# reglab/aquaculture

Hardware: AMD Instinct MI355X
Metric: 640px tiles/sec (whole node) YOLOv5m bf16 (higher is better)
Workload: dtype bf16

## Files before the change

aquaculture_amd/csrc/conv1x1_direct.hip:

```cpp
#include "conv_device.h"

using namespace aqdev;

namespace {

struct C1Params {
    const char* in;
    char* out;
    const char* w;
    const float* bias;
    const char* zero;
    int in_ld_b, out_ld_b;
    int npix, n_tiles, act;
    float out_inv_scale;
};

constexpr int kNW = 12;

template <int KS, int MBT, int MBW, int NBW> struct C1Geom {
    static constexpr int CIN = 32 * KS, COUT = 16 * MBT, CB = CIN / 8;
    static constexpr int MG = MBT / MBW;
    static constexpr int PG = kNW / MG;
    static constexpr int TP = PG * NBW * 16;
    static constexpr int SPP = CB + 2;
    static constexpr int PXB = SPP * 16;
    static constexpr int NQ = (TP * SPP + 63) / 64;
    static constexpr int XPB = NQ * 1024;
    static constexpr int LDS = 2 * XPB + COUT * 4;
    static constexpr int NST = NBW;
    static_assert(MBT % MBW == 0 && kNW % MG == 0 && LDS <= 160 * 1024, "shape");
};

__device__ __forceinline__ f32x4 c1_silu4(f32x4 v) {
    const f32x4 t = v * -1.44269504f;
    f32x4 d = {__builtin_amdgcn_exp2f(t[0]), __builtin_amdgcn_exp2f(t[1]), __builtin_amdgcn_exp2f(t[2]), __builtin_amdgcn_exp2f(t[3])};
    d = d + 1.0f;
    const f32x4 r = {__builtin_amdgcn_rcpf(d[0]), __builtin_amdgcn_rcpf(d[1]), __builtin_amdgcn_rcpf(d[2]), __builtin_amdgcn_rcpf(d[3])};
    return v * r;
}

template <int KS, int MBT, int MBW, int NBW, bool F8OUT = false>
__global__ __launch_bounds__(kNW * 64) void conv1x1_direct_kernel(const C1Params p) {
    using G = C1Geom<KS, MBT, MBW, NBW>;
    extern __shared__ __attribute__((aligned(16))) char smem[];
    float* s_b = (float*)(smem + 2 * G::XPB);

    const int tid = threadIdx.x, lane = tid & 63;
    const int wave = __builtin_amdgcn_readfirstlane(tid >> 6);
    static_assert(MBW == 2, "the paired-row layout below is written for two M blocks per wave");
    const int mb0 = (wave % G::MG) * MBW, pg = wave / G::MG;
    const int g = lane >> 4, l15 = lane & 15;
    const int cbase = mb0 * 16 + g * 8;

    bf16x8 wv[KS][MBW];
#pragma unroll
    for (int s = 0; s < KS; ++s)
#pragma unroll
        for (int m = 0; m < MBW; ++m) wv[s][m] = ((const bf16x8*)p.w)[((size_t)(mb0 + m) * KS + s) * 64 + lane];
    for (int i = tid; i < G::COUT; i += kNW * 64) s_b[i] = p.bias[i];

    auto issue_dma = [&](int tile, char* xb) {
        const long long n0 = (long long)tile * G::TP;
#pragma unroll 1
        for (int q = wave; q < G::NQ; q += kNW) {
            const int slot = q * 64 + lane;
            const int px = slot / G::SPP, part = slot - px * G::SPP;
            const bool valid = px < G::TP && part < G::CB && n0 + px < p.npix;
            const char* src = p.in + (n0 + px) * p.in_ld_b + part * 16;
            glds16(valid ? src : p.zero, xb + q * 1024);
        }
    };

    int tile = first_tile(gridDim.x, blockIdx.x);
    if (tile < p.n_tiles) issue_dma(tile, smem);
    int cur = 0;
    bool prev_full = false;
    for (; tile < p.n_tiles; tile += gridDim.x, cur ^= 1) {
        const long long n0 = (long long)tile * G::TP;
        const char* s_x = smem + cur * G::XPB;
        if (prev_full) wait_vmcnt<G::NST>(); else wait_vmcnt<0>();
        asm volatile("s_waitcnt lgkmcnt(0)" ::: "memory");
        __builtin_amdgcn_s_barrier();
        asm volatile("" ::: "memory");
        prev_full = n0 + G::TP <= p.npix;
        if (tile + (int)gridDim.x < p.n_tiles) issue_dma(tile + (int)gridDim.x, smem + (cur ^ 1) * G::XPB);

        f32x4 bv[MBW];
#pragma unroll
        for (int m = 0; m < MBW; ++m) bv[m] = *(const f32x4*)(s_b + cbase + m * 4);
        static_assert(G::NST == NBW * 1, "one 16-byte (8-byte with F8OUT) store per pixel block: the wait at the top of the tile loop counts these");
        AQ_STORE_LOOP_UNROLL
// ... 11 lines not shown
#pragma unroll
                for (int m = 0; m < MBW; ++m) acc[m] = __builtin_amdgcn_mfma_f32_16x16x32_bf16(wv[s][m], f[s], acc[m], 0, 0, 0);
            f32x4 v0 = acc[0] + bv[0], v1 = acc[1] + bv[1];
            if (p.act) { v0 = c1_silu4(v0); v1 = c1_silu4(v1); }
            if constexpr (F8OUT) {
                f32x4 q0 = v0 * p.out_inv_scale, q1 = v1 * p.out_inv_scale;
#pragma unroll
                for (int e = 0; e < 4; ++e) {
                    q0[e] = __builtin_amdgcn_fmed3f(q0[e], -448.0f, 448.0f);
                    q1[e] = __builtin_amdgcn_fmed3f(q1[e], -448.0f, 448.0f);
                }
                int w0 = __builtin_amdgcn_cvt_pk_fp8_f32(q0[0], q0[1], 0, false);
                w0 = __builtin_amdgcn_cvt_pk_fp8_f32(q0[2], q0[3], w0, true);
                int w1 = __builtin_amdgcn_cvt_pk_fp8_f32(q1[0], q1[1], 0, false);
                w1 = __builtin_amdgcn_cvt_pk_fp8_f32(q1[2], q1[3], w1, true);
                if (n0 + px < p.npix) *(uint2*)(p.out + (n0 + px) * p.out_ld_b + cbase) = make_uint2((unsigned)w0, (unsigned)w1);
            } else if (n0 + px < p.npix)
                *(uint4*)(p.out + (n0 + px) * p.out_ld_b + cbase * 2) =
                    make_uint4(pack_bf16x2(v0[0], v0[1]), pack_bf16x2(v0[2], v0[3]), pack_bf16x2(v1[0], v1[1]), pack_bf16x2(v1[2], v1[3]));
        }
    }
}

template <int KS, int MBT, int MBW, int NBW, bool F8OUT = false>
int launch_c1(C1Params p, hipStream_t stream) {
    using G = C1Geom<KS, MBT, MBW, NBW>;
    auto fn = conv1x1_direct_kernel<KS, MBT, MBW, NBW, F8OUT>;
    int cus = 0;
    AQ_CHECK_HIP(aq_kernel_lds((const void*)fn, G::LDS));
    AQ_CHECK_HIP(aq_cus(&cus));
    p.n_tiles = (p.npix + G::TP - 1) / G::TP;
    long long grid = cus;
    if (grid > p.n_tiles) grid = p.n_tiles;
    hipLaunchKernelGGL(fn, dim3((unsigned)grid), dim3(kNW * 64), G::LDS, stream, p);
    AQ_CHECK_HIP(hipGetLastError());
    return AQ_OK;
}

}

extern "C" int aq_conv1x1_direct_supported(int cin, int cout) {
    return (cin == 96 && cout == 96) || (cin == 192 && cout == 192) || (cin == 384 && (cout == 192 || cout == 384));
}

extern "C" int aq_pack_conv1x1_direct(const float* w_host, int cin, int cout, void* packed_dev, size_t* bytes, void* stream) {
    AQ_REQUIRE(w_host && bytes && aq_conv1x1_direct_supported(cin, cout), "pack_conv1x1_direct: unsupported %d -> %d", cin, cout);
    const int ks = cin / 32, mbt = cout / 16;
    *bytes = (size_t)mbt * ks * 64 * 16;
    if (!packed_dev) return AQ_OK;
    bf16_t* host = (bf16_t*)calloc(1, *bytes);
    AQ_REQUIRE(host, "pack_conv1x1_direct: out of host memory");
    for (int mb = 0; mb < mbt; ++mb)
        for (int s = 0; s < ks; ++s)
            for (int lane = 0; lane < 64; ++lane) {
                const int r = lane & 15, g = lane >> 4;
                const int co = (mb >> 1) * 32 + 8 * (r >> 2) + 4 * (mb & 1) + (r & 3);
                bf16_t* dst = host + (((size_t)mb * ks + s) * 64 + lane) * 8;
                for (int e = 0; e < 8; ++e) dst[e] = aq_f2bf(w_host[(size_t)co * cin + 32 * s + 8 * g + e]);
            }
// ... 5 lines not shown
}

extern "C" int aq_conv1x1_direct(const void* in_dev, int in_ld, int in_choff, void* out_dev, int out_ld, int out_choff, int cin, int cout,
                                 const void* packed_w_dev, const float* bias_dev, long long npix, int act, void* stream) {
    AQ_REQUIRE(in_dev && out_dev && packed_w_dev && bias_dev, "conv1x1_direct: null pointer");
    AQ_REQUIRE(aq_conv1x1_direct_supported(cin, cout), "conv1x1_direct: unsupported %d -> %d", cin, cout);
    AQ_REQUIRE(npix > 0 && npix < (1LL << 31), "conv1x1_direct: bad pixel count");
    AQ_REQUIRE(in_ld % 8 == 0 && out_ld % 8 == 0 && in_choff % 8 == 0 && out_choff % 8 == 0 && in_choff + cin <= in_ld && out_choff + cout <= out_ld,
               "conv1x1_direct: channel slices must be 8-aligned and inside their rows");
    C1Params p{};
    p.in = (const char*)in_dev + (size_t)in_choff * 2; p.in_ld_b = in_ld * 2;
    p.out = (char*)out_dev + (size_t)out_choff * 2; p.out_ld_b = out_ld * 2;
    p.w = (const char*)packed_w_dev; p.bias = bias_dev;
    p.npix = (int)npix; p.act = act;
    p.zero = aq_zero_page();
    AQ_REQUIRE(p.zero, "conv1x1_direct: zero page allocation failed");
    const hipStream_t st = (hipStream_t)stream;
    if (cin == 96) return launch_c1<3, 6, 2, 4>(p, st);
    if (cin == 192) return launch_c1<6, 12, 2, 4>(p, st);
    if (cout == 192) return launch_c1<12, 12, 2, 2>(p, st);
    return launch_c1<12, 24, 2, 4>(p, st);
}


extern "C" int aq_conv1x1_direct_f8out(const void* in_dev, int in_ld, int in_choff, void* out_dev, int out_pitch_bytes, int out_byte_off, int cin,
                                       int cout, const void* packed_w_dev, const float* bias_dev, long long npix, int act, float out_scale,
                                       void* stream) {
    AQ_REQUIRE(in_dev && out_dev && packed_w_dev && bias_dev, "conv1x1_direct_f8out: null pointer");
    AQ_REQUIRE((cin == 192 && cout == 192) || (cin == 384 && cout == 384), "conv1x1_direct_f8out: unsupported %d -> %d", cin, cout);
    AQ_REQUIRE(npix > 0 && npix < (1LL << 31) && out_scale > 0.0f, "conv1x1_direct_f8out: bad pixel count or scale");
    AQ_REQUIRE(in_ld % 8 == 0 && in_choff % 8 == 0 && in_choff + cin <= in_ld && out_pitch_bytes % 8 == 0 && out_byte_off % 8 == 0 &&
                   out_byte_off + cout <= out_pitch_bytes, "conv1x1_direct_f8out: slices must be 8-byte aligned and inside their rows");
    C1Params p{};
    p.in = (const char*)in_dev + (size_t)in_choff * 2; p.in_ld_b = in_ld * 2;
    p.out = (char*)out_dev + out_byte_off; p.out_ld_b = out_pitch_bytes;
    p.w = (const char*)packed_w_dev; p.bias = bias_dev;
    p.npix = (int)npix; p.act = act; p.out_inv_scale = 1.0f / out_scale;
    p.zero = aq_zero_page();
    AQ_REQUIRE(p.zero, "conv1x1_direct_f8out: zero page allocation failed");
    const hipStream_t st = (hipStream_t)stream;
    if (cin == 192) return launch_c1<6, 12, 2, 4, true>(p, st);
    return launch_c1<12, 24, 2, 4, true>(p, st);
}
```

aquaculture_amd/csrc/engine.cpp:

```cpp
#include "aq_common.h"
#include <unistd.h>
#include <string>

#include <cstdarg>
#include <cstdio>
#include <cstdlib>
#include <cstring>
#include <string>
#include <atomic>
#include <dlfcn.h>
#include <vector>

namespace {
thread_local char g_err[512] = "";
}

void aq_set_error(const char* fmt, ...) {
    va_list ap;
    va_start(ap, fmt);
    vsnprintf(g_err, sizeof(g_err), fmt, ap);
    va_end(ap);
}

extern "C" const char* aq_last_error(void) { return g_err; }
// ... 25 lines not shown
        return push && pop;
    }
} g_roctx;

constexpr int kCountStride = 1024;

struct PackedW {
    void* w = nullptr;
    float* bias = nullptr;
    int kgroups = 0, kgroups_pad = 0, G = 0, cout_rows = 0;
    bool x3 = false;
    void* w_direct = nullptr;
    int direct_cfg = -1;
    void* w_head = nullptr;
    void* w_pl8 = nullptr;
    float* sb_pl8 = nullptr;
    void* w_f8 = nullptr;
    float* sb_f8 = nullptr;
    float act_scale = 0.0f;
    int f8_consumer = -1;
    std::vector<float> w_host, b_host;
    void* w_tail = nullptr;
    float* b_tail = nullptr;
};

void pack_host(const float* w, int cout, int k, int cin, int precision, std::vector<unsigned char>& out,
               int* kgroups, int* kgroups_pad, int* G, int* cout_rows) {
    const int eb = aq_elem_bytes(precision);
    const int g = cin * eb / 16;
    const int kg = k * k * g;
    const int kgp = (kg + 7) / 8 * 8;
    const int rows = (cout + kCoutSlack + 31) / 32 * 32;
    out.assign((size_t)rows * kgp * 16, 0);
    const int kelems = k * k * cin;
    for (int co = 0; co < cout; ++co) {
        unsigned char* dst = out.data() + (size_t)co * kgp * 16;
        const float* src = w + (size_t)co * kelems;
        if (precision == AQ_FP32) {
            memcpy(dst, src, (size_t)kelems * 4);
        } else {
            bf16_t* d = (bf16_t*)dst;
            for (int e = 0; e < kelems; ++e) d[e] = aq_f2bf(src[e]);
        }
    }
    *kgroups = kg; *kgroups_pad = kgp; *G = g; *cout_rows = rows;
}
// ... 376 lines not shown
        }
        default:
            break;
        }
    }
    return -1;
}

bool c3tail_active(aq_engine* e, int oi, int last, int B) {
    if (!e->packed[oi].w_tail || oi + 1 >= last || e->calib_amax || e->tuning) return false;
    const int ci = oi + 1;
    const PackedW& pc = e->packed[ci];
    if (pc.direct_cfg != AQ_CONV_CFG_DIRECT1X1 || (pc.f8_consumer >= 0 && f8_pair_active(e, pc.f8_consumer, B))) return false;
    const aq_engine::Tuned* tt = tuned_for(e);
    const int cfg = e->conv_cfg[ci] >= 0 ? e->conv_cfg[ci] : tt ? tt->cfg[ci] : -1;
    if (cfg != AQ_CONV_CFG_DIRECT1X1) return false;
    const aq_op_desc& b = e->ops[oi];
    const aq_op_desc& c = e->ops[ci];
    const TensorPlace& pl = e->place[b.src.tensor];
    return aq_bottleneck_c3tail_supported(B, pl.h, pl.w, e->tensors[b.src.tensor].channels, e->tensors[c.src.tensor].channels,
                                          e->tensors[c.dst.tensor].channels) != 0;
}

struct AugRun {
    int pass;
    const aq_augment_pass* ps;
    int H0, W0;
    const aq_tap* ytab;
    const aq_tap* xtab;
};

int run_plan(aq_engine* e, const uint8_t* tiles, int B, int H, int W, void* ws, size_t ws_bytes,
             float* pred_out, aq_det* dets, int32_t* counts, float conf, float iou, int max_det, hipStream_t stream,
             int first = 0, int last = -1, const AugRun* ar = nullptr) {
    AQ_REQUIRE(e && tiles && ws, "infer: null pointer");
    const int n_ops = (int)e->ops.size();
    if (last < 0) last = n_ops;
    AQ_REQUIRE(0 <= first && first <= last && last <= n_ops, "run_ops: range [%d, %d) is not inside the plan's %d ops", first, last, n_ops);
    int rc = AQ_OK;
    if (!ar) {
        rc = layout(e, B, H, W);
        if (rc) return rc;
        if (ws_bytes < e->total_bytes) {
            aq_set_error("workspace too small: need %zu bytes, got %zu", e->total_bytes, ws_bytes);
            return AQ_ERR_WORKSPACE;
        }
// ... 3 lines not shown
    const float aug_scale = ar ? ar->ps->scale : 1.0f, aug_flip_w = ar && ar->ps->flip ? (float)ar->W0 : 0.0f;
    e->last_ws = ws; e->last_tiles = tiles;
    const int prec = e->desc.precision;
    const bool whole = first == 0 && last == n_ops;
    hipEvent_t* ev = nullptr;
    if (whole && !ar && e->prof && e->ring > 0) ev = e->ev.data() + (size_t)(e->prof_calls % e->ring) * (n_ops + 1);
    float* pred = pred_out ? pred_out : (float*)((char*)ws + e->off_pred);
    int32_t* cand = (int32_t*)((char*)ws + e->off_cand);
    int32_t* cand_count = (int32_t*)((char*)ws + e->off_cand_count);
    float* cand_rows = (float*)((char*)ws + e->off_cand_rows);
    const char* use_sd = getenv("AQ_STEMDOWN");
    const bool stemdown = use_sd && *use_sd == '1' && prec == AQ_BF16 && n_ops > 2 && e->ops[0].kind == AQ_OP_STEM && e->ops[1].kind == AQ_OP_DOWNBLOCK &&
                          e->ops[0].dst.channels == 48 && e->ops[1].src.tensor == e->ops[0].dst.tensor && e->ops[1].src.ch_off == e->ops[0].dst.ch_off &&
                          aq_stemdown_supported(H, W) && ((uintptr_t)tiles & 3) == 0 && !scaled;
    const bool fuse_heads = dets != nullptr && heads_fused(e);
    bool heads_started = ar != nullptr;
    int heads_done = 0;
    for (int oi = 0; oi < first; ++oi)
        if (fuse_heads && e->ops[oi].kind == AQ_OP_CONV && e->ops[oi].level >= 0) {
            heads_started = true;
            ++heads_done;
        }
    int tail_conv = -1;
    for (int oi = first; oi < last; ++oi) {
        const aq_op_desc& op = e->ops[oi];
        if (ev) AQ_CHECK_HIP(hipEventRecord(ev[oi], stream));
        const bool mark = g_roctx.on();
        if (mark) {
            char name[96];
            snprintf(name, sizeof name, "aq op %02d kind %d: %d -> %d ch, k%d s%d%s", oi, op.kind, op.src.channels, op.dst.channels, op.k, op.stride,
                     op.level >= 0 ? " (detect head)" : "");
            g_roctx.push(name);
        }
        switch (op.kind) {
        case AQ_OP_PREPROCESS:
            if (scaled)
                rc = aq_preprocess_s2d_scaled(tiles, ar->H0, ar->W0, ar->ytab, ar->xtab, ar->ps->h, ar->ps->w, tptr(e, ws, tiles, op.dst.tensor), B, H, W,
                                              prec, stream);
            else
                rc = aq_preprocess_s2d(tiles, tptr(e, ws, tiles, op.dst.tensor), B, H, W, prec, stream);
            break;
        case AQ_OP_CONV:
            if (oi == tail_conv) {
                note_launch(e, oi, AQ_FAM_DIRECT1X1, AQ_CONV_CFG_DIRECT1X1);
                break;
            }
            if (ar && op.level >= 0 && !((ar->ps->level_mask >> op.level) & 1)) {
                note_launch(e, oi, AQ_FAM_NONE);
                break;
            }
            if (fuse_heads && op.level >= 0) {
                int32_t* wide = (int32_t*)((char*)ws + e->off_cand_wide);
                if (!heads_started) {
                    AQ_CHECK_HIP(hipMemsetAsync(wide, 0, sizeof(int32_t) * B * kCountStride, stream));
                    heads_started = true;
                }
                const TensorPlace& pl = e->place[op.src.tensor];
                int off = 0;
                for (int l = 0; l < op.level; ++l) off += e->desc.na * (H / (int)e->desc.stride[l]) * (W / (int)e->desc.stride[l]);
                float anchors[8 * 2];
                for (int a = 0; a < e->desc.na; ++a) {
                    anchors[2 * a] = e->desc.anchors_px[op.level][a][0];
                    anchors[2 * a + 1] = e->desc.anchors_px[op.level][a][1];
                }
                note_launch(e, oi, AQ_FAM_HEAD_DECODE);
                if (ar) {
                    rc = aq_head_decode_aug(tptr(e, ws, tiles, op.src.tensor), e->tensors[op.src.tensor].channels, op.src.ch_off, op.src.channels,
// ... 45 lines not shown
                               op.src.channels, e->packed[oi].w, e->packed[oi].bias, B, pl.h, pl.w, op.res.tensor >= 0, stream);
            break;
        }
        case AQ_OP_DOWNBLOCK: {
            note_launch(e, oi, AQ_FAM_DOWNBLOCK);
            const TensorPlace& pl = e->place[op.src.tensor];
            if (stemdown && oi == 1) {
                rc = aq_stemdown(tiles, tptr(e, ws, tiles, op.dst.tensor), e->tensors[op.dst.tensor].channels, op.dst.ch_off,
                                 e->packed[0].w, e->packed[0].bias, e->packed[oi].w, e->packed[oi].bias, B, H, W, stream);
                break;
            }
            rc = aq_downblock(tptr(e, ws, tiles, op.src.tensor), e->tensors[op.src.tensor].channels, op.src.ch_off,
                              tptr(e, ws, tiles, op.dst.tensor), e->tensors[op.dst.tensor].channels, op.dst.ch_off,
                              e->packed[oi].w, e->packed[oi].bias, B, pl.h, pl.w, stream);
            break;
        }
        case AQ_OP_SPPF_POOL: {
            const TensorPlace& pl = e->place[op.src.tensor];
            rc = aq_sppf_pool(tptr(e, ws, tiles, op.src.tensor), e->tensors[op.src.tensor].channels, op.src.ch_off,
                              op.src.channels, B, pl.h, pl.w, prec, stream);
            break;
        }
        case AQ_OP_UPSAMPLE2X: {
            const TensorPlace& pl = e->place[op.src.tensor];
            rc = aq_upsample2x(tptr(e, ws, tiles, op.src.tensor), e->tensors[op.src.tensor].channels, op.src.ch_off,
                               tptr(e, ws, tiles, op.dst.tensor), e->tensors[op.dst.tensor].channels, op.dst.ch_off,
                               op.src.channels, B, pl.h, pl.w, prec, stream);
            break;
        }
        case AQ_OP_DECODE: {
            if (fuse_heads) break;
            const float* heads[3];
            for (int l = 0; l < 3; ++l) heads[l] = (const float*)tptr(e, ws, tiles, e->desc.head_tensor[l]);
            float anchors[3 * 8 * 2];
            for (int l = 0; l < 3; ++l)
                for (int a = 0; a < e->desc.na; ++a) {
                    anchors[(l * e->desc.na + a) * 2] = e->desc.anchors_px[l][a][0];
                    anchors[(l * e->desc.na + a) * 2 + 1] = e->desc.anchors_px[l][a][1];
                }
            const bool want_nms = dets != nullptr;
            if (ar) {
                rc = aq_detect_decode_aug(heads, e->tensors[e->desc.head_tensor[0]].channels, B, H, W, e->desc.nc, e->desc.na, anchors,
                                          e->desc.stride, ar->ps->level_mask, aug_base, e->N, aug_scale, aug_flip_w, want_nms ? nullptr : pred,
                                          conf, want_nms ? cand : nullptr, want_nms ? cand_rows : nullptr, want_nms ? cand_count : nullptr,
                                          e->N, stream);
                break;
// ... 370 lines not shown
                        (void)hipFree(pw.w_pl8); (void)hipFree(pw.sb_pl8);
                        pw.w_pl8 = nullptr; pw.sb_pl8 = nullptr;
                    }
                }
            }
        }
        const char* no_hf = getenv("AQ_DISABLE_HEAD_FUSION");
        if (d->precision == AQ_BF16 && op.level >= 0 && op.k == 1 && op.stride == 1 && !op.act && op.res.tensor < 0 &&
            op.dst.channels >= d->na * (d->nc + 5) && op.dst.channels <= 32 && aq_head_decode_supported(op.src.channels, d->na, d->nc) && !(no_hf && *no_hf == '1')) {
            size_t nb = 0;
            if (aq_pack_head_weights(op.weight, op.bias, op.src.channels, op.dst.channels, nullptr, &nb, nullptr) != AQ_OK ||
                hipMalloc(&pw.w_head, nb) != hipSuccess ||
                aq_pack_head_weights(op.weight, op.bias, op.src.channels, op.dst.channels, pw.w_head, &nb, nullptr) != AQ_OK) {
                aq_set_error("engine_create: fused head weight upload failed (op %zu)", oi);
                return fail(AQ_ERR_HIP);
            }
        }
        if (d->precision == AQ_BF16 && op.kind == AQ_OP_CONV && op.k == 3 && op.stride == 1 && op.pad == 1 && e->packed[oi].direct_cfg == AQ_CONV_CFG_PL3X3 &&
            aq_conv3x3_pl_f8_supported(op.src.channels, op.dst.channels, 1, 8, 8)) {
            e->packed[oi].w_host.assign(op.weight, op.weight + (size_t)op.dst.channels * 9 * op.src.channels);
            e->packed[oi].b_host.assign(op.bias, op.bias + op.dst.channels);
        }
        op.weight = nullptr; op.bias = nullptr;
    }
    *out = e;
    return AQ_OK;
}

extern "C" void aq_engine_destroy(aq_engine* e) {
    if (!e) return;
    for (PackedW& pw : e->packed) {
        if (pw.w) (void)hipFree(pw.w);
        if (pw.w_direct) (void)hipFree(pw.w_direct);
        if (pw.w_head) (void)hipFree(pw.w_head);
        if (pw.w_pl8) (void)hipFree(pw.w_pl8);
        if (pw.w_f8) (void)hipFree(pw.w_f8);
        if (pw.sb_f8) (void)hipFree(pw.sb_f8);
        if (pw.sb_pl8) (void)hipFree(pw.sb_pl8);
        if (pw.w_tail) (void)hipFree(pw.w_tail);
        if (pw.b_tail) (void)hipFree(pw.b_tail);
        if (pw.bias) (void)hipFree(pw.bias);
    }
    if (e->zero_page) (void)hipFree(e->zero_page);
    for (hipEvent_t ev : e->ev) (void)hipEventDestroy(ev);
    delete e;
}
// ... 328 lines not shown
```

aquaculture_amd/engine.py:

```python
from __future__ import annotations

import ctypes as C
import os
import re
from typing import Dict, List, Optional, Sequence, Tuple

import numpy as np
import torch

from . import spec as _spec
from .checkpoint import Checkpoint, pack_plan_weights

AQ_BF16, AQ_FP32, AQ_BF16_W8, AQ_F16X3 = 0, 1, 2, 3
PRECISIONS = {"bf16": AQ_BF16, "fp32": AQ_FP32, "fp8w": AQ_BF16, "f16x3": AQ_F16X3}
"""Compute precision of the single-op helpers.  fp8w = fp8 (OCP e4m3fn) weights with per-output-channel power-of-two scales, bf16
activations (quant.py): values bf16 holds exactly, so every bf16 kernel runs them as they are."""
ENGINE_PRECISIONS = {"bf16": AQ_BF16, "fp32": AQ_FP32, "fp8w": AQ_BF16_W8, "f16x3": AQ_F16X3, "fp8": AQ_BF16}
"""aq_model_desc.precision.  AQ_BF16_W8 computes as AQ_BF16; kernels with an fp8-weight stream (the planar 3x3) load the e4m3 codes."""
_DTYPE_CODE = {"act": 0, "f32": 1, "u8": 2}

LIB_PATH = os.path.join(os.path.dirname(os.path.abspath(__file__)), "csrc", "libaqengine.so")


class aq_tensor_desc(C.Structure):
# ... 9 lines not shown
                ("k", C.c_int32), ("stride", C.c_int32), ("pad", C.c_int32), ("act", C.c_int32),
                ("level", C.c_int32), ("weight", C.POINTER(C.c_float)), ("bias", C.POINTER(C.c_float)),
                ("flops_per_tile", C.c_double)]


class aq_model_desc(C.Structure):
    _fields_ = [("precision", C.c_int32), ("nc", C.c_int32), ("na", C.c_int32), ("nl", C.c_int32),
                ("anchors_px", C.c_float * 2 * 8 * 3), ("stride", C.c_float * 3),
                ("head_tensor", C.c_int32 * 3), ("input_tensor", C.c_int32),
                ("n_tensors", C.c_int32), ("n_ops", C.c_int32),
                ("tensors", C.POINTER(aq_tensor_desc)), ("ops", C.POINTER(aq_op_desc))]


class aq_det(C.Structure):
    _fields_ = [("x1", C.c_float), ("y1", C.c_float), ("x2", C.c_float), ("y2", C.c_float),
                ("conf", C.c_float), ("cls", C.c_float)]


EXPORTS = (
    "aq_last_error", "aq_version", "aq_engine_create", "aq_engine_destroy", "aq_engine_workspace_bytes",
    "aq_engine_infer", "aq_engine_run_ops", "aq_engine_candidates", "aq_engine_forward_raw", "aq_engine_tensor_ptr", "aq_engine_profile",
    "aq_engine_op_times", "aq_engine_num_ops", "aq_engine_set_conv_config", "aq_engine_autotune", "aq_engine_set_tuned_table",
    "aq_engine_get_conv_config", "aq_conv_num_configs", "aq_debug_conv_stamp", "aq_debug_mfma_peak",
    "aq_conv_config_tiles", "aq_pack_conv_weights", "aq_pack_conv_weights_x3", "aq_conv2d", "aq_pack_stem_weights", "aq_stem_conv", "aq_pack_bottleneck_weights", "aq_bottleneck", "aq_bottleneck_asm_form", "aq_bottleneck_c3tail_supported", "aq_pack_bottleneck_c3tail_weights", "aq_bottleneck_c3tail", "aq_pack_downblock_weights", "aq_downblock", "aq_stemdown_supported", "aq_stemdown", "aq_conv1x1_direct_supported", "aq_pack_conv1x1_direct", "aq_conv1x1_direct", "aq_conv1x1_asm_supported", "aq_pack_conv1x1_asm", "aq_conv1x1_asm", "aq_nms_opts", "aq_engine_set_nms_options",
    "aq_conv3x3s2_direct_supported", "aq_pack_conv3x3s2_direct", "aq_conv3x3s2_direct",
    "aq_conv3x3_pl_supported", "aq_conv3x3_pl_asm_family", "aq_pack_conv3x3_pl", "aq_conv3x3_pl", "aq_conv3x3_pl_s2_supported", "aq_pack_conv3x3_pl_s2", "aq_conv3x3_pl_s2", "aq_jpeg_scratch_bytes", "aq_jpeg_idct_rgb", "aq_f32_to_e4m3", "aq_conv1x1_direct_f8out", "aq_absmax_bf16", "aq_engine_calibrate_amax", "aq_engine_set_fp8_scales", "aq_engine_last_launch", "aq_conv3x3_pl_f8_supported", "aq_pack_conv3x3_pl_f8", "aq_conv3x3_pl_f8", "aq_conv3x3_pl_w8_supported", "aq_pack_conv3x3_pl_w8", "aq_conv3x3_pl_w8", "aq_head_decode_supported", "aq_pack_head_weights", "aq_head_decode", "aq_head_counts_gather", "aq_preprocess_s2d", "aq_sppf_pool",
    "aq_upsample2x", "aq_letterbox_u8", "aq_letterbox_tiles_u8", "aq_format_label_rows", "aq_detect_decode", "aq_nms_scratch_bytes", "aq_nms", "aq_jpeg_huffman_decode", "aq_write_label_files",
    "aq_crop_jpeg_coefs", "aq_crop_jpeg_bytes", "aq_write_crop_files",
    "aq_annotate_u8", "aq_image_jpeg_coefs", "aq_image_jpeg_bytes", "aq_write_image_files",
    "aq_blank_stats_scratch_bytes", "aq_blank_stats_u8",
    "aq_augment_geometry", "aq_augment_taps", "aq_stem_conv_scaled", "aq_preprocess_s2d_scaled", "aq_head_decode_aug", "aq_detect_decode_aug",
    "aq_engine_workspace_bytes_augment", "aq_engine_infer_augment", "aq_engine_forward_raw_augment", "aq_engine_last_launch_augment",
)

_lib = None


def load_library(path: str = LIB_PATH) -> C.CDLL:
    global _lib
    if _lib is not None:
        return _lib
    if path == LIB_PATH and os.environ.get("AQ_ENGINE_LIB"):
        path = os.environ["AQ_ENGINE_LIB"]
    if not os.path.exists(path):
        raise RuntimeError(f"{path} not found: build it with `python -m aquaculture_amd.build` "
                           "(there is no CPU/PyTorch fallback for the detect path)")
    lib = C.CDLL(path)
# ... 37 lines not shown
    lib.aq_engine_set_fp8_scales.argtypes = [vp, C.POINTER(f32), i32]
    lib.aq_conv1x1_direct_f8out.argtypes = [vp, i32, i32, vp, i32, i32, i32, i32, vp, vp, C.c_longlong, i32, f32, vp]
    lib.aq_absmax_bf16.argtypes = [vp, i32, i32, i32, C.c_longlong, vp, vp]
    lib.aq_debug_conv_stamp.argtypes = [vp, sz]
    lib.aq_debug_mfma_peak.argtypes = [i32, i32, vp, vp]
    lib.aq_conv_config_tiles.argtypes = [i32, C.POINTER(i32), C.POINTER(i32)]
    lib.aq_pack_conv_weights.argtypes = [C.POINTER(f32), i32, i32, i32, i32, vp, C.POINTER(sz), vp]
    lib.aq_pack_conv_weights_x3.argtypes = [C.POINTER(f32), C.POINTER(f32), i32, i32, i32, vp, C.POINTER(sz), vp, C.POINTER(sz), vp]
    lib.aq_conv2d.argtypes = [vp, i32, i32, i32, vp, i32, i32, i32, vp, i32, i32, vp, vp,
                              i32, i32, i32, i32, i32, i32, i32, i32, i32, vp, vp]
    lib.aq_pack_stem_weights.argtypes = [C.POINTER(f32), i32, i32, vp, C.POINTER(sz), vp]
    lib.aq_stem_conv.argtypes = [vp, vp, i32, i32, i32, vp, vp, i32, i32, i32, i32, i32, vp]
    lib.aq_pack_bottleneck_weights.argtypes = [C.POINTER(f32), C.POINTER(f32), i32, vp, C.POINTER(sz), vp]
    lib.aq_bottleneck.argtypes = [vp, i32, i32, vp, i32, i32, i32, vp, vp, i32, i32, i32, i32, vp]
    lib.aq_bottleneck_asm_form.argtypes = [i32] * 6
    lib.aq_bottleneck_c3tail_supported.argtypes = [i32, i32, i32, i32, i32, i32]
    lib.aq_pack_bottleneck_c3tail_weights.argtypes = [C.POINTER(f32), C.POINTER(f32), C.POINTER(f32), vp, C.POINTER(sz), vp]
    lib.aq_bottleneck_c3tail.argtypes = [vp, i32, i32, vp, i32, i32, vp, i32, i32, vp, vp, i32, i32, i32, i32, vp]
    lib.aq_pack_downblock_weights.argtypes = [C.POINTER(f32), C.POINTER(f32), vp, C.POINTER(sz), vp]
    lib.aq_downblock.argtypes = [vp, i32, i32, vp, i32, i32, vp, vp, i32, i32, i32, vp]
    lib.aq_conv1x1_direct_supported.argtypes = [i32, i32]
    lib.aq_pack_conv1x1_direct.argtypes = [C.POINTER(f32), i32, i32, vp, C.POINTER(sz), vp]
    lib.aq_conv1x1_direct.argtypes = [vp, i32, i32, vp, i32, i32, i32, i32, vp, vp, C.c_longlong, i32, vp]
    lib.aq_nms_opts.argtypes = [vp, i32, i32, i32, i32, f32, f32, i32, vp, vp, i32, vp, vp, vp, i32, C.c_ulonglong, C.c_ulonglong, vp]
    lib.aq_engine_set_nms_options.argtypes = [vp, i32, C.c_ulonglong, C.c_ulonglong]
    lib.aq_conv1x1_asm_supported.argtypes = [i32, i32]
    lib.aq_pack_conv1x1_asm.argtypes = [C.POINTER(f32), i32, i32, vp, C.POINTER(sz), vp]
    lib.aq_conv1x1_asm.argtypes = [vp, i32, i32, vp, i32, i32, i32, i32, vp, vp, C.c_longlong, i32, vp]
    lib.aq_conv3x3s2_direct_supported.argtypes = [i32, i32]
    lib.aq_pack_conv3x3s2_direct.argtypes = [C.POINTER(f32), i32, i32, vp, C.POINTER(sz), vp]
    lib.aq_conv3x3s2_direct.argtypes = [vp, i32, i32, vp, i32, i32, i32, i32, vp, vp, i32, i32, i32, i32, vp]
    lib.aq_conv3x3_pl_supported.argtypes = [i32, i32]
    lib.aq_conv3x3_pl_asm_family.argtypes = [i32]
    lib.aq_pack_conv3x3_pl.argtypes = [C.POINTER(f32), i32, i32, vp, C.POINTER(sz), vp]
    lib.aq_conv3x3_pl.argtypes = [vp, C.c_longlong, C.c_longlong, i32, vp, i32, i32, i32, vp, i32, i32, vp, vp, i32, i32, i32, i32, vp]
    lib.aq_conv3x3_pl_w8.argtypes = lib.aq_conv3x3_pl.argtypes
    lib.aq_pack_conv3x3_pl_w8.argtypes = [C.POINTER(C.c_float), C.POINTER(C.c_float), i32, i32, vp, C.POINTER(C.c_size_t), vp, vp]
    lib.aq_conv3x3_pl_w8_supported.argtypes = [i32] * 5
    lib.aq_jpeg_scratch_bytes.argtypes = [i32, i32, i32]
    lib.aq_jpeg_scratch_bytes.restype = sz
    lib.aq_jpeg_idct_rgb.argtypes = [vp, vp, vp, i32, i32, i32, vp, vp, vp]
    lib.aq_f32_to_e4m3.argtypes = [f32]
    lib.aq_f32_to_e4m3.restype = C.c_ubyte
    lib.aq_conv3x3_pl_f8_supported.argtypes = [i32] * 5
    lib.aq_pack_conv3x3_pl_f8.argtypes = [C.POINTER(f32), C.POINTER(f32), i32, i32, f32, vp, C.POINTER(sz), vp, vp]
    lib.aq_conv3x3_pl_f8.argtypes = [vp, i32, i32, i32, vp, i32, i32, i32, vp, i32, i32, vp, vp, i32, i32, i32, i32, vp]
# ... 969 lines not shown

def conv1x1_direct_nhwc(x: torch.Tensor, w_oihw: torch.Tensor, bias: torch.Tensor, act: bool = True, out: Optional[torch.Tensor] = None) -> torch.Tensor:
    _require_gpu()
    lib = load_library()
    assert x.dtype == torch.bfloat16 and x.stride(-1) == 1
    cin, cout = x.shape[-1], w_oihw.shape[0]
    ld = x.stride(-2)
    npix = x.numel() // cin
    w = np.ascontiguousarray(w_oihw.reshape(cout, cin).float().cpu().numpy())
    n = C.c_size_t()
    wp = w.ctypes.data_as(C.POINTER(C.c_float))
    _check(lib.aq_pack_conv1x1_direct(wp, cin, cout, None, C.byref(n), None))
    wbuf = torch.empty(n.value, dtype=torch.uint8, device=x.device)
    _check(lib.aq_pack_conv1x1_direct(wp, cin, cout, wbuf.data_ptr(), C.byref(n), _stream_ptr()))
    bbuf = bias.float().to(x.device).contiguous()
    if out is None:
        out = torch.empty(x.shape[:-1] + (cout,), dtype=torch.bfloat16, device=x.device)
    _check(lib.aq_conv1x1_direct(x.data_ptr(), ld, 0, out.data_ptr(), out.stride(-2), 0, cin, cout, wbuf.data_ptr(), bbuf.data_ptr(), npix, int(act),
                                 _stream_ptr()))
    torch.cuda.current_stream().synchronize()
    return out


def conv1x1_asm_nhwc(x: torch.Tensor, w_oihw: torch.Tensor, bias: torch.Tensor, out: Optional[torch.Tensor] = None) -> torch.Tensor:
    _require_gpu()
    lib = load_library()
    assert x.dtype == torch.bfloat16 and x.stride(-1) == 1
    cin, cout = x.shape[-1], w_oihw.shape[0]
    ld = x.stride(-2)
    npix = x.numel() // cin
    w = np.ascontiguousarray(w_oihw.reshape(cout, cin).float().cpu().numpy())
    n = C.c_size_t()
    wp = w.ctypes.data_as(C.POINTER(C.c_float))
    _check(lib.aq_pack_conv1x1_asm(wp, cin, cout, None, C.byref(n), None))
    wbuf = torch.empty(n.value, dtype=torch.uint8, device=x.device)
    _check(lib.aq_pack_conv1x1_asm(wp, cin, cout, wbuf.data_ptr(), C.byref(n), _stream_ptr()))
    bbuf = bias.float().to(x.device).contiguous()
    if out is None:
        out = torch.empty(x.shape[:-1] + (cout,), dtype=torch.bfloat16, device=x.device)
    _check(lib.aq_conv1x1_asm(x.data_ptr(), ld, 0, out.data_ptr(), out.stride(-2), 0, cin, cout, wbuf.data_ptr(), bbuf.data_ptr(), npix, 1, _stream_ptr()))
    torch.cuda.current_stream().synchronize()
    return out


def conv3x3s2_direct_nhwc(x: torch.Tensor, w_oihw: torch.Tensor, bias: torch.Tensor, act: bool = True, out: Optional[torch.Tensor] = None) -> torch.Tensor:
    _require_gpu()
# ... 252 lines not shown
```

include/aq_engine.h:

```cpp
#ifndef AQ_ENGINE_H
#define AQ_ENGINE_H

#include <stddef.h>
#include <stdint.h>

#ifdef __cplusplus
extern "C" {
#endif

typedef enum aq_status {
    AQ_OK = 0,
    AQ_ERR_INVALID = -1,
    AQ_ERR_HIP = -2,
    AQ_ERR_NOMEM = -3,
    AQ_ERR_WORKSPACE = -4
} aq_status;

typedef enum aq_precision {
    AQ_BF16 = 0,
    AQ_FP32 = 1,
    AQ_BF16_W8 = 2,
    AQ_F16X3 = 3
} aq_precision;

// ... 108 lines not shown
                  const void* packed_w_dev, const float* bias_dev, int B, int H, int W, int shortcut, void* stream);
int aq_bottleneck_asm_form(int C, int B, int H, int W, int in_ld, int out_ld);

int aq_bottleneck_c3tail_supported(int B, int H, int W, int in_ld, int cat_ld, int out_ld);
int aq_pack_bottleneck_c3tail_weights(const float* w1_host, const float* w2_host, const float* w3_host, void* packed_dev, size_t* bytes,
                                      void* stream);
int aq_bottleneck_c3tail(const void* in_dev, int in_ld, int in_choff, const void* cat_dev, int cat_ld, int cat_choff, void* out_dev,
                         int out_ld, int out_choff, const void* packed_w_dev, const float* bias_dev, int B, int H, int W, int shortcut,
                         void* stream);

int aq_pack_downblock_weights(const float* wa_host, const float* wb_host, void* packed_dev, size_t* bytes, void* stream);
int aq_downblock(const void* in_dev, int in_ld, int in_choff, void* out_dev, int out_ld, int out_choff,
                 const void* packed_w_dev, const float* bias_dev, int B, int H, int W, void* stream);
int aq_stemdown_supported(int Hi, int Wi);
int aq_stemdown(const uint8_t* tiles_dev, void* out_dev, int out_ld, int out_choff, const void* stem_w_dev, const float* stem_bias_dev,
                const void* packed_w_dev, const float* bias_dev, int B, int Hi, int Wi, void* stream);

#define AQ_CONV_CFG_DIRECT1X1 1000
#define AQ_CONV_CFG_ONE_TILE_PER_WG 4096
int aq_conv1x1_direct_supported(int cin, int cout);
int aq_pack_conv1x1_direct(const float* w_host, int cin, int cout, void* packed_dev, size_t* bytes, void* stream);
int aq_conv1x1_direct(const void* in_dev, int in_ld, int in_choff, void* out_dev, int out_ld, int out_choff, int cin, int cout,
                      const void* packed_w_dev, const float* bias_dev, long long npix, int act, void* stream);

#define AQ_CONV_CFG_ASM1X1 1004
int aq_conv1x1_asm_supported(int cin, int cout);
int aq_pack_conv1x1_asm(const float* w_host, int cin, int cout, void* packed_dev, size_t* bytes, void* stream);
int aq_conv1x1_asm(const void* in_dev, int in_ld, int in_choff, void* out_dev, int out_ld, int out_choff, int cin, int cout,
                   const void* packed_w_dev, const float* bias_dev, long long npix, int act, void* stream);

#define AQ_CONV_CFG_DIRECT3X3S2 1001
int aq_conv3x3s2_direct_supported(int cin, int cout);
int aq_pack_conv3x3s2_direct(const float* w_host, int cin, int cout, void* packed_dev, size_t* bytes, void* stream);
int aq_conv3x3s2_direct(const void* in_dev, int in_ld, int in_choff, void* out_dev, int out_ld, int out_choff, int cin, int cout,
                        const void* packed_w_dev, const float* bias_dev, int B, int H, int W, int act, void* stream);
#define AQ_CONV_CFG_PL3X3 1002
int aq_conv3x3_pl_supported(int cin, int cout);
int aq_conv3x3_pl_asm_family(int nb);
int aq_pack_conv3x3_pl(const float* w_krsc_host, int cin, int cout, void* packed_dev, size_t* bytes, void* stream);
int aq_conv3x3_pl(const void* in_dev, long long in_pixel_stride_b, long long in_group_stride_b, int cin,
                  void* out_dev, int out_ld, int out_choff, int cout, const void* res_dev, int res_ld, int res_choff,
                  const void* packed_w_dev, const float* bias_dev, int B, int H, int W, int act, void* stream);
#define AQ_CONV_CFG_PL3X3S2 1003
int aq_conv3x3_pl_s2_supported(int cin, int cout, int B, int H, int W);
int aq_pack_conv3x3_pl_s2(const float* w_krsc_host, int cin, int cout, void* packed_dev, size_t* bytes, void* stream);
int aq_conv3x3_pl_s2(const void* in_dev, int in_ld, int in_choff, int cin, void* out_dev, int out_ld, int out_choff, int cout,
// ... 117 lines not shown
```

Before: 17110.

## Fuse nearest 2x upsample into following direct 1x1 conv input gather

Adds an UP2X variant of the direct 1x1 conv kernel that reads the upsampled half of its concatenated input straight from the low-resolution tensor. It computes source coordinates with magic-number division inside the DMA issue loop. The engine detects upsample→1x1 conv pairs whose upsampled output is read by nothing else, skips the upsample launch and calls the fused kernel instead. This removes one kernel launch plus the write and re-read of the upsampled tensor per pair, at the cost of extra integer arithmetic and less contiguous loads in the prefetch loop.

```diff
diff --git a/aquaculture_amd/csrc/conv1x1_direct.hip b/aquaculture_amd/csrc/conv1x1_direct.hip
--- a/aquaculture_amd/csrc/conv1x1_direct.hip
+++ b/aquaculture_amd/csrc/conv1x1_direct.hip
@@ -13,6 +13,9 @@
     int in_ld_b, out_ld_b;
     int npix, n_tiles, act;
     float out_inv_scale;
+    const char* lo;
+    int lo_ld_b, lo_parts;
+    unsigned hw, hw_mul, hw_sh, wd, wd_mul, wd_sh, h2, w2;
 };
 
 constexpr int kNW = 12;
@@ -39,7 +42,7 @@
     return v * r;
 }
 
-template <int KS, int MBT, int MBW, int NBW, bool F8OUT = false>
+template <int KS, int MBT, int MBW, int NBW, bool F8OUT = false, bool UP2X = false>
 __global__ __launch_bounds__(kNW * 64) void conv1x1_direct_kernel(const C1Params p) {
     using G = C1Geom<KS, MBT, MBW, NBW>;
     extern __shared__ __attribute__((aligned(16))) char smem[];
@@ -67,6 +70,15 @@
             const int px = slot / G::SPP, part = slot - px * G::SPP;
             const bool valid = px < G::TP && part < G::CB && n0 + px < p.npix;
             const char* src = p.in + (n0 + px) * p.in_ld_b + part * 16;
+            if constexpr (UP2X) {
+                if (part < p.lo_parts) {
+                    const unsigned n = (unsigned)(n0 + px);
+                    const unsigned b = __umulhi(n, p.hw_mul) >> p.hw_sh, r = n - b * p.hw;
+                    const unsigned y = __umulhi(r, p.wd_mul) >> p.wd_sh, x = r - y * p.wd;
+                    src = p.lo + (long long)((b * p.h2 + (y >> 1)) * p.w2 + (x >> 1)) * p.lo_ld_b + part * 16;
+                } else
+                    src -= p.lo_parts * 16;
+            }
             glds16(valid ? src : p.zero, xb + q * 1024);
         }
     };
@@ -124,10 +136,10 @@
     }
 }
 
-template <int KS, int MBT, int MBW, int NBW, bool F8OUT = false>
+template <int KS, int MBT, int MBW, int NBW, bool F8OUT = false, bool UP2X = false>
 int launch_c1(C1Params p, hipStream_t stream) {
     using G = C1Geom<KS, MBT, MBW, NBW>;
-    auto fn = conv1x1_direct_kernel<KS, MBT, MBW, NBW, F8OUT>;
+    auto fn = conv1x1_direct_kernel<KS, MBT, MBW, NBW, F8OUT, UP2X>;
     int cus = 0;
     AQ_CHECK_HIP(aq_kernel_lds((const void*)fn, G::LDS));
     AQ_CHECK_HIP(aq_cus(&cus));
@@ -137,6 +149,13 @@
     hipLaunchKernelGGL(fn, dim3((unsigned)grid), dim3(kNW * 64), G::LDS, stream, p);
     AQ_CHECK_HIP(hipGetLastError());
     return AQ_OK;
+}
+
+void c1_magic(unsigned d, unsigned* mul, unsigned* sh) {
+    unsigned l = 1;
+    while ((1ull << l) < d) ++l;
+    *mul = (unsigned)(((1ull << (31 + l)) + d - 1) / d);
+    *sh = l - 1;
 }
 
 }
@@ -188,6 +207,37 @@
     return launch_c1<12, 24, 2, 4>(p, st);
 }
 
+extern "C" int aq_conv1x1_direct_up2x_supported(int c_lo, int cin, int cout, int B, int H, int W) {
+    return aq_conv1x1_direct_supported(cin, cout) && c_lo % 8 == 0 && 0 < c_lo && c_lo < cin && B > 0 && H > 0 && W > 0 && H % 2 == 0 && W % 2 == 0 &&
+           (long long)B * H * W < (1LL << 31);
+}
+
+extern "C" int aq_conv1x1_direct_up2x(const void* lo_dev, int lo_ld, int lo_choff, int c_lo, const void* skip_dev, int skip_ld, int skip_choff,
+                                      void* out_dev, int out_ld, int out_choff, int cin, int cout, const void* packed_w_dev, const float* bias_dev,
+                                      int B, int H, int W, int act, void* stream) {
+    AQ_REQUIRE(lo_dev && skip_dev && out_dev && packed_w_dev && bias_dev, "conv1x1_direct_up2x: null pointer");
+    AQ_REQUIRE(aq_conv1x1_direct_up2x_supported(c_lo, cin, cout, B, H, W), "conv1x1_direct_up2x: unsupported %d + %d -> %d at %d x %d x %d", c_lo,
+               cin - c_lo, cout, B, H, W);
+    AQ_REQUIRE(lo_ld % 8 == 0 && skip_ld % 8 == 0 && out_ld % 8 == 0 && lo_choff % 8 == 0 && skip_choff % 8 == 0 && out_choff % 8 == 0 &&
+                   lo_choff >= 0 && skip_choff >= 0 && out_choff >= 0 && lo_choff + c_lo <= lo_ld && skip_choff + cin - c_lo <= skip_ld &&
+                   out_choff + cout <= out_ld, "conv1x1_direct_up2x: channel slices must be 8-aligned and inside their rows");
+    C1Params p{};
+    p.lo = (const char*)lo_dev + (size_t)lo_choff * 2; p.lo_ld_b = lo_ld * 2; p.lo_parts = c_lo / 8;
+    p.in = (const char*)skip_dev + (size_t)skip_choff * 2; p.in_ld_b = skip_ld * 2;
+    p.out = (char*)out_dev + (size_t)out_choff * 2; p.out_ld_b = out_ld * 2;
+    p.w = (const char*)packed_w_dev; p.bias = bias_dev;
+    p.npix = (int)((long long)B * H * W); p.act = act;
+    p.hw = (unsigned)H * (unsigned)W; p.wd = (unsigned)W; p.h2 = (unsigned)H / 2; p.w2 = (unsigned)W / 2;
+    c1_magic(p.hw, &p.hw_mul, &p.hw_sh);
+    c1_magic(p.wd, &p.wd_mul, &p.wd_sh);
+    p.zero = aq_zero_page();
+    AQ_REQUIRE(p.zero, "conv1x1_direct_up2x: zero page allocation failed");
+    const hipStream_t st = (hipStream_t)stream;
+    if (cin == 96) return launch_c1<3, 6, 2, 4, false, true>(p, st);
+    if (cin == 192) return launch_c1<6, 12, 2, 4, false, true>(p, st);
+    if (cout == 192) return launch_c1<12, 12, 2, 2, false, true>(p, st);
+    return launch_c1<12, 24, 2, 4, false, true>(p, st);
+}
 
 extern "C" int aq_conv1x1_direct_f8out(const void* in_dev, int in_ld, int in_choff, void* out_dev, int out_pitch_bytes, int out_byte_off, int cin,
                                        int cout, const void* packed_w_dev, const float* bias_dev, long long npix, int act, float out_scale,
diff --git a/aquaculture_amd/csrc/engine.cpp b/aquaculture_amd/csrc/engine.cpp
--- a/aquaculture_amd/csrc/engine.cpp
+++ b/aquaculture_amd/csrc/engine.cpp
@@ -71,6 +71,7 @@
     std::vector<float> w_host, b_host;
     void* w_tail = nullptr;
     float* b_tail = nullptr;
+    bool up2x = false;
 };
 
 void pack_host(const float* w, int cout, int k, int cin, int precision, std::vector<unsigned char>& out,
@@ -493,6 +494,21 @@
                                           e->tensors[c.dst.tensor].channels) != 0;
 }
 
+bool up2x_active(aq_engine* e, int oi, int last, int B) {
+    if (!e->packed[oi].up2x || oi + 1 >= last || e->calib_amax || e->tuning) return false;
+    const int ci = oi + 1;
+    const PackedW& pc = e->packed[ci];
+    if (pc.direct_cfg != AQ_CONV_CFG_DIRECT1X1 || (pc.f8_consumer >= 0 && f8_pair_active(e, pc.f8_consumer, B))) return false;
+    const aq_engine::Tuned* tt = tuned_for(e);
+    const int cfg = e->conv_cfg[ci] >= 0 ? e->conv_cfg[ci] : tt ? tt->cfg[ci] : -1;
+    if (cfg != AQ_CONV_CFG_DIRECT1X1) return false;
+    const aq_op_desc& u = e->ops[oi];
+    const aq_op_desc& c = e->ops[ci];
+    const TensorPlace& pl = e->place[u.src.tensor];
+    const TensorPlace& pd = e->place[c.dst.tensor];
+    return pd.h == 2 * pl.h && pd.w == 2 * pl.w && aq_conv1x1_direct_up2x_supported(u.src.channels, c.src.channels, c.dst.channels, B, pd.h, pd.w) != 0;
+}
+
 struct AugRun {
     int pass;
     const aq_augment_pass* ps;
@@ -542,6 +558,7 @@
             ++heads_done;
         }
     int tail_conv = -1;
+    int up2x_conv = -1;
     for (int oi = first; oi < last; ++oi) {
         const aq_op_desc& op = e->ops[oi];
         if (ev) AQ_CHECK_HIP(hipEventRecord(ev[oi], stream));
@@ -563,6 +580,17 @@
         case AQ_OP_CONV:
             if (oi == tail_conv) {
                 note_launch(e, oi, AQ_FAM_DIRECT1X1, AQ_CONV_CFG_DIRECT1X1);
+                break;
+            }
+            if (oi == up2x_conv) {
+                const aq_op_desc& u = e->ops[oi - 1];
+                const TensorPlace& pd = e->place[op.dst.tensor];
+                note_launch(e, oi, AQ_FAM_DIRECT1X1, AQ_CONV_CFG_DIRECT1X1);
+                rc = aq_conv1x1_direct_up2x(tptr(e, ws, tiles, u.src.tensor), e->tensors[u.src.tensor].channels, u.src.ch_off, u.src.channels,
+                                            tptr(e, ws, tiles, op.src.tensor), e->tensors[op.src.tensor].channels, op.src.ch_off + u.dst.channels,
+                                            tptr(e, ws, tiles, op.dst.tensor), e->tensors[op.dst.tensor].channels, op.dst.ch_off,
+                                            op.src.channels, op.dst.channels, e->packed[oi].w_direct, e->packed[oi].bias, B, pd.h, pd.w, op.act,
+                                            stream);
                 break;
             }
             if (ar && op.level >= 0 && !((ar->ps->level_mask >> op.level) & 1)) {
@@ -654,6 +682,10 @@
             break;
         }
         case AQ_OP_UPSAMPLE2X: {
+            if (up2x_active(e, oi, last, B)) {
+                up2x_conv = oi + 1;
+                break;
+            }
             const TensorPlace& pl = e->place[op.src.tensor];
             rc = aq_upsample2x(tptr(e, ws, tiles, op.src.tensor), e->tensors[op.src.tensor].channels, op.src.ch_off,
                                tptr(e, ws, tiles, op.dst.tensor), e->tensors[op.dst.tensor].channels, op.dst.ch_off,
@@ -1070,6 +1102,24 @@
             e->packed[oi].b_host.assign(op.bias, op.bias + op.dst.channels);
         }
         op.weight = nullptr; op.bias = nullptr;
+    }
+    const char* use_up2x = getenv("AQ_UP2X");
+    for (size_t oi = 0; d->precision == AQ_BF16 && !(use_up2x && *use_up2x == '0') && oi + 1 < e->ops.size(); ++oi) {
+        const aq_op_desc& u = e->ops[oi];
+        const aq_op_desc& c = e->ops[oi + 1];
+        if (u.kind != AQ_OP_UPSAMPLE2X || c.kind != AQ_OP_CONV || e->packed[oi + 1].direct_cfg != AQ_CONV_CFG_DIRECT1X1) continue;
+        if (c.k != 1 || c.stride != 1 || c.res.tensor >= 0 || c.level >= 0 || c.src.tensor != u.dst.tensor || c.src.ch_off != u.dst.ch_off ||
+            c.src.channels != e->tensors[c.src.tensor].channels || u.dst.channels != u.src.channels || u.dst.channels >= c.src.channels ||
+            u.src.tensor == u.dst.tensor || c.dst.tensor == u.src.tensor || c.dst.tensor == c.src.tensor ||
+            e->tensors[u.src.tensor].dtype != AQ_T_ACT || e->tensors[c.src.tensor].dtype != AQ_T_ACT ||
+            e->tensors[u.dst.tensor].down * 2 != e->tensors[u.src.tensor].down || e->tensors[c.dst.tensor].down != e->tensors[c.src.tensor].down)
+            continue;
+        bool read_elsewhere = false;
+        for (size_t oj = 0; oj < e->ops.size(); ++oj)
+            for (const aq_slice* s : {&e->ops[oj].src, &e->ops[oj].res})
+                if (oj != oi + 1 && s->tensor == u.dst.tensor && s->ch_off < u.dst.ch_off + u.dst.channels && u.dst.ch_off < s->ch_off + s->channels)
+                    read_elsewhere = true;
+        e->packed[oi].up2x = !read_elsewhere;
     }
     *out = e;
     return AQ_OK;
diff --git a/aquaculture_amd/engine.py b/aquaculture_amd/engine.py
--- a/aquaculture_amd/engine.py
+++ b/aquaculture_amd/engine.py
@@ -55,7 +55,7 @@
     "aq_engine_infer", "aq_engine_run_ops", "aq_engine_candidates", "aq_engine_forward_raw", "aq_engine_tensor_ptr", "aq_engine_profile",
     "aq_engine_op_times", "aq_engine_num_ops", "aq_engine_set_conv_config", "aq_engine_autotune", "aq_engine_set_tuned_table",
     "aq_engine_get_conv_config", "aq_conv_num_configs", "aq_debug_conv_stamp", "aq_debug_mfma_peak",
-    "aq_conv_config_tiles", "aq_pack_conv_weights", "aq_pack_conv_weights_x3", "aq_conv2d", "aq_pack_stem_weights", "aq_stem_conv", "aq_pack_bottleneck_weights", "aq_bottleneck", "aq_bottleneck_asm_form", "aq_bottleneck_c3tail_supported", "aq_pack_bottleneck_c3tail_weights", "aq_bottleneck_c3tail", "aq_pack_downblock_weights", "aq_downblock", "aq_stemdown_supported", "aq_stemdown", "aq_conv1x1_direct_supported", "aq_pack_conv1x1_direct", "aq_conv1x1_direct", "aq_conv1x1_asm_supported", "aq_pack_conv1x1_asm", "aq_conv1x1_asm", "aq_nms_opts", "aq_engine_set_nms_options",
+    "aq_conv_config_tiles", "aq_pack_conv_weights", "aq_pack_conv_weights_x3", "aq_conv2d", "aq_pack_stem_weights", "aq_stem_conv", "aq_pack_bottleneck_weights", "aq_bottleneck", "aq_bottleneck_asm_form", "aq_bottleneck_c3tail_supported", "aq_pack_bottleneck_c3tail_weights", "aq_bottleneck_c3tail", "aq_pack_downblock_weights", "aq_downblock", "aq_stemdown_supported", "aq_stemdown", "aq_conv1x1_direct_supported", "aq_pack_conv1x1_direct", "aq_conv1x1_direct", "aq_conv1x1_direct_up2x_supported", "aq_conv1x1_direct_up2x", "aq_conv1x1_asm_supported", "aq_pack_conv1x1_asm", "aq_conv1x1_asm", "aq_nms_opts", "aq_engine_set_nms_options",
     "aq_conv3x3s2_direct_supported", "aq_pack_conv3x3s2_direct", "aq_conv3x3s2_direct",
     "aq_conv3x3_pl_supported", "aq_conv3x3_pl_asm_family", "aq_pack_conv3x3_pl", "aq_conv3x3_pl", "aq_conv3x3_pl_s2_supported", "aq_pack_conv3x3_pl_s2", "aq_conv3x3_pl_s2", "aq_jpeg_scratch_bytes", "aq_jpeg_idct_rgb", "aq_f32_to_e4m3", "aq_conv1x1_direct_f8out", "aq_absmax_bf16", "aq_engine_calibrate_amax", "aq_engine_set_fp8_scales", "aq_engine_last_launch", "aq_conv3x3_pl_f8_supported", "aq_pack_conv3x3_pl_f8", "aq_conv3x3_pl_f8", "aq_conv3x3_pl_w8_supported", "aq_pack_conv3x3_pl_w8", "aq_conv3x3_pl_w8", "aq_head_decode_supported", "aq_pack_head_weights", "aq_head_decode", "aq_head_counts_gather", "aq_preprocess_s2d", "aq_sppf_pool",
     "aq_upsample2x", "aq_letterbox_u8", "aq_letterbox_tiles_u8", "aq_format_label_rows", "aq_detect_decode", "aq_nms_scratch_bytes", "aq_nms", "aq_jpeg_huffman_decode", "aq_write_label_files",
@@ -139,6 +139,8 @@
     lib.aq_conv1x1_direct_supported.argtypes = [i32, i32]
     lib.aq_pack_conv1x1_direct.argtypes = [C.POINTER(f32), i32, i32, vp, C.POINTER(sz), vp]
     lib.aq_conv1x1_direct.argtypes = [vp, i32, i32, vp, i32, i32, i32, i32, vp, vp, C.c_longlong, i32, vp]
+    lib.aq_conv1x1_direct_up2x_supported.argtypes = [i32, i32, i32, i32, i32, i32]
+    lib.aq_conv1x1_direct_up2x.argtypes = [vp, i32, i32, i32, vp, i32, i32, vp, i32, i32, i32, i32, vp, vp, i32, i32, i32, i32, vp]
     lib.aq_nms_opts.argtypes = [vp, i32, i32, i32, i32, f32, f32, i32, vp, vp, i32, vp, vp, vp, i32, C.c_ulonglong, C.c_ulonglong, vp]
     lib.aq_engine_set_nms_options.argtypes = [vp, i32, C.c_ulonglong, C.c_ulonglong]
     lib.aq_conv1x1_asm_supported.argtypes = [i32, i32]
@@ -1154,6 +1156,43 @@
     return out
 
 
+def pack_conv1x1_direct(w_oihw: torch.Tensor, bias: torch.Tensor, device) -> Tuple[torch.Tensor, torch.Tensor]:
+    lib = load_library()
+    cout, cin = w_oihw.shape[0], w_oihw.shape[1]
+    w = np.ascontiguousarray(w_oihw.reshape(cout, cin).float().cpu().numpy())
+    n = C.c_size_t()
+    wp = w.ctypes.data_as(C.POINTER(C.c_float))
+    _check(lib.aq_pack_conv1x1_direct(wp, cin, cout, None, C.byref(n), None))
+    wbuf = torch.empty(n.value, dtype=torch.uint8, device=device)
+    _check(lib.aq_pack_conv1x1_direct(wp, cin, cout, wbuf.data_ptr(), C.byref(n), _stream_ptr()))
+    return wbuf, bias.float().to(device).contiguous()
+
+
+def conv1x1_direct_up2x_supported(c_lo: int, cin: int, cout: int, B: int, H: int, W: int) -> bool:
+    return bool(load_library().aq_conv1x1_direct_up2x_supported(c_lo, cin, cout, B, H, W))
+
+
+def conv1x1_direct_up2x_nhwc(lo: torch.Tensor, skip: torch.Tensor, packed: Tuple[torch.Tensor, torch.Tensor], act: bool = True,
+                             out: Optional[torch.Tensor] = None, sync: bool = True) -> torch.Tensor:
+    _require_gpu()
+    lib = load_library()
+    assert lo.dtype == torch.bfloat16 and skip.dtype == torch.bfloat16 and lo.stride(3) == 1 and skip.stride(3) == 1
+    B, H, W, c_skip = skip.shape
+    c_lo = lo.shape[3]
+    assert lo.shape[:3] == (B, H // 2, W // 2)
+    for t in (lo, skip):
+        assert t.stride(1) == t.shape[2] * t.stride(2) and t.stride(0) == t.shape[1] * t.stride(1), "channel slices of dense NHWC tensors"
+    cout = packed[1].numel()
+    if out is None:
+        out = torch.empty((B, H, W, cout), dtype=torch.bfloat16, device=skip.device)
+    assert out.stride(3) == 1 and out.stride(1) == W * out.stride(2) and out.stride(0) == H * out.stride(1)
+    _check(lib.aq_conv1x1_direct_up2x(lo.data_ptr(), lo.stride(2), 0, c_lo, skip.data_ptr(), skip.stride(2), 0, out.data_ptr(), out.stride(2), 0,
+                                      c_lo + c_skip, cout, packed[0].data_ptr(), packed[1].data_ptr(), B, H, W, int(act), _stream_ptr()))
+    if sync:
+        torch.cuda.current_stream().synchronize()
+    return out
+
+
 def conv1x1_asm_nhwc(x: torch.Tensor, w_oihw: torch.Tensor, bias: torch.Tensor, out: Optional[torch.Tensor] = None) -> torch.Tensor:
     _require_gpu()
     lib = load_library()
diff --git a/include/aq_engine.h b/include/aq_engine.h
--- a/include/aq_engine.h
+++ b/include/aq_engine.h
@@ -154,6 +154,10 @@
 int aq_pack_conv1x1_direct(const float* w_host, int cin, int cout, void* packed_dev, size_t* bytes, void* stream);
 int aq_conv1x1_direct(const void* in_dev, int in_ld, int in_choff, void* out_dev, int out_ld, int out_choff, int cin, int cout,
                       const void* packed_w_dev, const float* bias_dev, long long npix, int act, void* stream);
+int aq_conv1x1_direct_up2x_supported(int c_lo, int cin, int cout, int B, int H, int W);
+int aq_conv1x1_direct_up2x(const void* lo_dev, int lo_ld, int lo_choff, int c_lo, const void* skip_dev, int skip_ld, int skip_choff,
+                           void* out_dev, int out_ld, int out_choff, int cin, int cout, const void* packed_w_dev, const float* bias_dev,
+                           int B, int H, int W, int act, void* stream);
 
 #define AQ_CONV_CFG_ASM1X1 1004
 int aq_conv1x1_asm_supported(int cin, int cout);
```

Result: no change. 17170, median of 2 (+0.4%).
